# chongminggao/CIRS-codes

Hardware: AMD Instinct MI355X
Metric: simulator env-steps/s (collect + PPO update in the timed region), KuaishouEnv (higher is better)
Workload: dtype f32 (policy/tracker; rollout on the fp32 MFMA, PPO head products fp32-accurate from two fp16 pieces per operand (3 f16 MFMAs per product), fp32 accumulate) + f64 (env rewards, GAE)

## Files before the change

### cirs-codes_amd/csrc/internal.h

```cpp
#pragma once
#include "common.h"
#include "policy_kernels.h"

namespace cirs {

struct TrunkFuse {
    int on;
    cirs_policy_cfg cfg;
    cirs_policy_weights w;
    const uint8_t* skip;
    float* h2;
    float* value;
};

inline int device_cu_count() {
    static int cus = 0;
    if (cus == 0) {
        int dev = 0, n = 0;
        if (hipGetDevice(&dev) == hipSuccess && hipDeviceGetAttribute(&n, hipDeviceAttributeMultiprocessorCount, dev) == hipSuccess && n > 0) cus = n;
        else cus = 256;
    }
    return cus;
}

inline int head_tiles_per_chunk(int n_item_tiles, int n_row_blocks, int wgs_per_cu) {
    const long slots = (long)wgs_per_cu * device_cu_count();
    const int tpc = (int)(((long)n_item_tiles * n_row_blocks + slots - 1) / slots);
    return tpc < 4 ? 4 : tpc;
}

inline HeadGrid sampler_grid(int n_items, int n_pad) {
    HeadGrid g;
    const int tiles = (n_items + kTileN - 1) / kTileN;
    g.n_row_blocks = (n_pad / kTileM + 3) / 4;
    g.tiles_per_chunk = head_tiles_per_chunk(tiles, g.n_row_blocks, kSamplerWgsPerCu);
// ... 93 lines not shown
```

### cirs-codes_amd/csrc/policy.hip

```cpp
#include "policy_kernels.h"
#include "internal.h"

namespace cirs {

__global__ __launch_bounds__(256) void actor_merge_kernel(int n, int n_pad, int n_chunks, ActorPartialView pv,
                                                          const uint8_t* __restrict__ skip,
                                                          int64_t* __restrict__ act_out, float* __restrict__ logp_out) {
    const int lane = threadIdx.x & 63;
    const int j = blockIdx.x * 4 + (threadIdx.x >> 6);
    if (j >= n) return;
    if (skip && skip[j]) {
        if (lane == 0) {
            act_out[j] = -1;
            if (logp_out) logp_out[j] = 0.f;
        }
        return;
    }
    actor_merge_wave(j, lane, n_pad, n_chunks, pv, act_out, logp_out);
}

__global__ __launch_bounds__(256) void actor_shard_tuple_kernel(int n, int n_pad, int n_chunks, ActorPartialView pv,
                                                               const uint8_t* __restrict__ skip, float* __restrict__ out5) {
    const int lane = threadIdx.x & 63;
    const int j = blockIdx.x * 4 + (threadIdx.x >> 6);
// ... 92 lines not shown
    const long k = (long)blockIdx.x * blockDim.x + threadIdx.x;
    if (k >= n * q) return;
    const long r = k / q;
    const int c = (int)(k - r * q);
    const long id = idx[r];
    reinterpret_cast<float4*>(out)[k] = id < 0 ? make_float4(0.f, 0.f, 0.f, 0.f) : reinterpret_cast<const float4*>(table + (size_t)id * row_floats)[c];
}

static int validate_policy(const cirs_policy_cfg* cfg, const cirs_policy_weights* w) {
    CIRS_REQUIRE(cfg && w, "policy cfg/weights null");
    CIRS_REQUIRE(cfg->n_items > 0, "n_items must be positive");
    if (cfg->hidden != kH) return fail(CIRS_E_UNSUPPORTED, "this build supports hidden == 64 only");
    CIRS_REQUIRE(cfg->dim_state > 0 && cfg->dim_state <= 64, "dim_state must be in 1..64");
    CIRS_REQUIRE(w->w1 && w->b1 && w->w2 && w->b2 && w->wa && w->ba && w->wc && w->bc, "policy weight pointer null");
    return CIRS_OK;
}

}

extern "C" int64_t cirs_policy_workspace_bytes(const cirs_policy_cfg* cfg, int32_t n) {
    using namespace cirs;
    if (!cfg || n <= 0) return 0;
    return (int64_t)(ws_h2_floats(n) + 5 * ws_partial_elems(n, cfg->n_items) + ws_zstore_floats(n, cfg->n_items)) * 4 + 8192 + kTrkImgBytes +
           (int64_t)ws_rplanes_bytes(cfg->n_items) + 512;
}

extern "C" int cirs_actor_sample(const cirs_policy_cfg* cfg, const cirs_policy_weights* w, const float* state,
                                 int64_t state_stride, int32_t n, const float* gumbel, uint64_t seed,
                                 uint32_t rng_step, const int32_t* env_ids, const uint32_t* visited,
                                 const uint8_t* skip, int64_t* act_out, float* logp_out, float* value_out,
                                 void* workspace, int64_t workspace_bytes, void* stream) {
    using namespace cirs;
    if (int rc = validate_policy(cfg, w)) return rc;
    if (n <= 0) return CIRS_OK;
    CIRS_REQUIRE(state && act_out && workspace, "null state/act/workspace");
    CIRS_REQUIRE(state_stride >= cfg->dim_state, "state_stride < dim_state");
    if (n <= 0) return CIRS_OK;
    CIRS_REQUIRE(workspace_bytes >= cirs_policy_workspace_bytes(cfg, n), "workspace too small");
    hipStream_t s = (hipStream_t)stream;
    float* h2 = (float*)workspace;
    const int n_pad = n_pad_of(n);
    const HeadGrid hg = sampler_grid(cfg->n_items, n_pad);
    const int n_chunks = hg.n_chunks;
    ActorPartialView pv = partial_view(workspace, n, cfg->n_items);
    hipLaunchKernelGGL(trunk_kernel, dim3(cdiv(n, 4)), dim3(256), 0, s, *cfg, *w, state, (long)state_stride, n, skip, h2,
                       value_out, nullptr);
    CIRS_CHECK_LAUNCH("trunk_kernel");
    if (!gumbel) {
        const int nch = n_chunks_of(cfg->n_items);
        const int cpw = mass_chunks_per_wg(nch, hg.n_row_blocks);
        uint4* planes = ws_rplanes(workspace, workspace_bytes, cfg->n_items);
        if (int rc = build_rplanes(w->wa, cfg->n_items, planes, s)) return rc;
        hipLaunchKernelGGL(actor_mass_kernel, dim3(cdiv(nch, cpw), hg.n_row_blocks), dim3(kMassThreads), 0, s, *cfg, (const uint4*)planes, w->ba, (const float*)h2, n,
                           env_ids, visited, skip, pv.m, n_pad, cpw, 0, 0);
        CIRS_CHECK_LAUNCH("actor_mass_kernel");
        PickArgs pa{pv.m, n_pad, nch, w->wa, w->ba, h2, visited, cfg->n_items, 0, 0, seed, rng_step};
        hipLaunchKernelGGL(actor_pick_kernel, dim3(cdiv(n, 4)), dim3(256), 0, s, pa, n, env_ids, skip, act_out, logp_out, (float*)nullptr);
        CIRS_CHECK_LAUNCH("actor_pick_kernel");
        return CIRS_OK;
    }
    const dim3 grid(hg.grid_x, hg.n_row_blocks);
    hipLaunchKernelGGL(actor_head_kernel<kNoiseHarness>, grid, dim3(256), 0, s, *cfg, w->wa, w->ba, h2, n, gumbel, seed,
                       rng_step, env_ids, visited, skip, pv, n_pad, hg.tiles_per_chunk);
    CIRS_CHECK_LAUNCH("actor_head_kernel");
    hipLaunchKernelGGL(actor_merge_kernel, dim3(cdiv(n, 4)), dim3(256), 0, s, n, n_pad, n_chunks, pv, skip, act_out, logp_out);
    CIRS_CHECK_LAUNCH("actor_merge_kernel");
    return CIRS_OK;
}

namespace cirs {
static int greedy_head(const cirs_policy_cfg* cfg, const cirs_policy_weights* w, const float* state, int64_t state_stride, int32_t n,
                       const int32_t* env_ids, const uint32_t* visited, const uint8_t* skip, float* value_out, void* workspace, float* zfull,
                       hipStream_t s) {
    float* h2 = (float*)workspace;
    const int n_pad = n_pad_of(n);
    const HeadGrid hg = sampler_grid(cfg->n_items, n_pad);
// ... 75 lines not shown
                                         int64_t state_stride, int32_t n, uint64_t seed, uint32_t rng_step, const int32_t* env_ids,
                                         const uint32_t* visited, const uint8_t* skip, int32_t item_base, int32_t n_items_total,
                                         float* tuples_out, float* value_out, void* workspace, int64_t workspace_bytes, void* stream) {
    using namespace cirs;
    if (int rc = validate_policy(cfg_shard, w_shard)) return rc;
    if (n <= 0) return CIRS_OK;
    CIRS_REQUIRE(state && tuples_out && workspace, "null state/tuples/workspace");
    CIRS_REQUIRE(state_stride >= cfg_shard->dim_state, "state_stride < dim_state");
    CIRS_REQUIRE(item_base >= 0 && (item_base % CIRS_SAMPLER_CHUNK) == 0, "item_base must be a non-negative multiple of the sampler chunk (128 items)");
    CIRS_REQUIRE(n_items_total >= item_base + cfg_shard->n_items, "n_items_total < item_base + shard size");
    CIRS_REQUIRE(workspace_bytes >= cirs_policy_workspace_bytes(cfg_shard, n), "workspace too small");
    hipStream_t s = (hipStream_t)stream;
    float* h2 = (float*)workspace;
    const int n_pad = n_pad_of(n);
    const HeadGrid hg = sampler_grid(cfg_shard->n_items, n_pad);
    ActorPartialView pv = partial_view(workspace, n, cfg_shard->n_items);
    hipLaunchKernelGGL(trunk_kernel, dim3(cdiv(n, 4)), dim3(256), 0, s, *cfg_shard, *w_shard, state, (long)state_stride, n, skip, h2,
                       value_out, nullptr);
    CIRS_CHECK_LAUNCH("trunk_kernel");
    const int nch = n_chunks_of(cfg_shard->n_items);
    const int cpw = mass_chunks_per_wg(nch, hg.n_row_blocks);
    uint4* planes = ws_rplanes(workspace, workspace_bytes, cfg_shard->n_items);
    if (int rc = build_rplanes(w_shard->wa, cfg_shard->n_items, planes, s)) return rc;
    hipLaunchKernelGGL(actor_mass_kernel, dim3(cdiv(nch, cpw), hg.n_row_blocks), dim3(kMassThreads), 0, s, *cfg_shard, (const uint4*)planes, w_shard->ba,
                       (const float*)h2, n, env_ids, visited, skip, pv.m, n_pad, cpw, item_base, n_items_total);
    CIRS_CHECK_LAUNCH("actor_mass_kernel");
    PickArgs pa{pv.m, n_pad, nch, w_shard->wa, w_shard->ba, h2, visited, cfg_shard->n_items, item_base, n_items_total, seed, rng_step};
    hipLaunchKernelGGL(actor_pick_kernel, dim3(cdiv(n, 4)), dim3(256), 0, s, pa, n, env_ids, skip, (int64_t*)nullptr, (float*)nullptr, tuples_out);
    CIRS_CHECK_LAUNCH("actor_pick_kernel");
    return CIRS_OK;
}

extern "C" int cirs_actor_merge_shards(const float* tuples, int32_t n_shards, int32_t n, const uint8_t* skip, int64_t* act_out,
                                       float* logp_out, void* stream) {
    using namespace cirs;
    if (n <= 0) return CIRS_OK;
    CIRS_REQUIRE(tuples && act_out && n_shards > 0, "null tuples / act_out or n_shards <= 0");
    hipLaunchKernelGGL(actor_merge_shards_kernel, dim3(cdiv(n, 256)), dim3(256), 0, (hipStream_t)stream, tuples, n_shards, n, skip,
                       act_out, logp_out);
    CIRS_CHECK_LAUNCH("actor_merge_shards_kernel");
    return CIRS_OK;
}

extern "C" int cirs_gather_rows(const float* table, int32_t row_floats, const int64_t* idx, int64_t n, float* out, void* stream) {
    using namespace cirs;
    if (n <= 0) return CIRS_OK;
    CIRS_REQUIRE(table && idx && out, "null argument");
// ... 7 lines not shown
```

### cirs-codes_amd/csrc/policy_kernels.h

```cpp
#pragma once
#include "bf16x6.h"
#include "common.h"
#include "rng.h"

namespace cirs {

constexpr int kH = 64;
constexpr int kTileM = 32;
constexpr int kTileN = 32;
constexpr int kTilesPerChunk = 4;
constexpr int kChunkItems = kTileN * kTilesPerChunk;

typedef float f32x16 __attribute__((ext_vector_type(16)));

struct ActorPartialView {
    float* score;
    int32_t* idx;
    float* m;
    float* s;
    float* z;
};

__host__ __device__ inline int n_chunks_of(int n_items) { return (n_items + kChunkItems - 1) / kChunkItems; }
__host__ __device__ inline int n_pad_of(int n) { return ((n + kTileM - 1) / kTileM) * kTileM; }
// ... 283 lines not shown

constexpr int kMassRowB = 144;
constexpr int kMassPlaneB = kTileN * kMassRowB;
constexpr int kMassTileU4 = 512;
constexpr int kMassThreads = 512;
constexpr float kMassScWa = 256.f, kMassScH2 = 64.f, kMassScZ = kMassScWa * kMassScH2, kMassScZi = 1.0f / kMassScZ;
__host__ __device__ inline size_t ws_rplanes_bytes(int n_items) { return (size_t)n_chunks_of(n_items) * kTilesPerChunk * kMassTileU4 * 16; }

static __global__ __launch_bounds__(256) void wa_rplanes_kernel(const float* __restrict__ wa, int I, uint4* __restrict__ planes) {
    const int tid = threadIdx.x, tile = blockIdx.x;
    const int item = tile * kTileN + (tid >> 3), col = 8 * (tid & 7);
    typedef float rp_v4 __attribute__((ext_vector_type(4)));
    rp_v4 a = {0.f, 0.f, 0.f, 0.f}, b = a;
    if (item < I) {
        const rp_v4* src = reinterpret_cast<const rp_v4*>(wa + (size_t)item * kH + col);
        a = src[0]; b = src[1];
    }
    a *= kMassScWa; b *= kMassScWa;
    const Planes2 pl = split8h(a.x, a.y, a.z, a.w, b.x, b.y, b.z, b.w);
    uint4* out = planes + (size_t)tile * kMassTileU4;
    out[tid] = __builtin_bit_cast(uint4, pl.h); out[256 + tid] = __builtin_bit_cast(uint4, pl.l);
}

__device__ __forceinline__ void mass_split_hidden(const float* tile, int lo, int hi, Planes2 (&hz)[4]) {
    typedef float ms_v4 __attribute__((ext_vector_type(4)));
#pragma unroll
    for (int s4 = 0; s4 < 4; ++s4) {
        const ms_v4* src = reinterpret_cast<const ms_v4*>(&tile[lo * kLdsStride + 16 * s4 + 8 * hi]);
        const ms_v4 a = src[0] * kMassScH2, b = src[1] * kMassScH2;
        hz[s4] = split8h(a.x, a.y, a.z, a.w, b.x, b.y, b.z, b.w);
    }
}
__device__ __forceinline__ f32x16 mass_logits_tile(const unsigned char* tw, const float* sb, const Planes2 (&hz)[4], int lo, int hi) {
    Planes2 za[4];
#pragma unroll
    for (int s4 = 0; s4 < 4; ++s4) {
        const unsigned char* ap = tw + lo * kMassRowB + (16 * s4 + 8 * hi) * 2;
        za[s4].h = *reinterpret_cast<const f16x8*>(ap);
        za[s4].l = *reinterpret_cast<const f16x8*>(ap + kMassPlaneB);
    }
    f32x16 acc, accs, acct;
#pragma unroll
    for (int r = 0; r < 16; ++r) { acc[r] = sb[acc_row(r, hi)]; accs[r] = 0.f; acct[r] = 0.f; }
    mfma_f16x3_split2(za[0], hz[0], za[1], hz[1], acc, accs, acct);
    mfma_f16x3_split2(za[2], hz[2], za[3], hz[3], acc, accs, acct);
#pragma unroll
    for (int r = 0; r < 16; ++r) acc[r] = (acc[r] + (accs[r] + acct[r])) * kMassScZi;
    return acc;
}
__device__ __forceinline__ float mass_exp(float z, float nml) { return __builtin_amdgcn_exp2f(__builtin_fmaf(z, 1.4426950408889634f, nml)); }
__device__ __forceinline__ float mass_log(float s) { return __builtin_amdgcn_logf(s) * 0.6931471805599453f; }

#ifdef CIRS_MASS_PROF
static __device__ unsigned long long g_mass_prof[32];
#define CIRS_MSTAMP(K) do { if (blockIdx.x == 0 && blockIdx.y == 0 && threadIdx.x == 0) g_mass_prof[K] = __builtin_amdgcn_s_memtime(); } while (0)
#define CIRS_MSTAMP_IF(COND, K) do { if ((COND) && blockIdx.x == 0 && blockIdx.y == 0 && threadIdx.x == 0) g_mass_prof[K] = __builtin_amdgcn_s_memtime(); } while (0)
#else
#define CIRS_MSTAMP(K) do { } while (0)
#define CIRS_MSTAMP_IF(COND, K) do { } while (0)
#endif
static __global__ __launch_bounds__(512, 1) void actor_mass_kernel(cirs_policy_cfg cfg, const uint4* __restrict__ planes,
                                                                   const float* __restrict__ ba, const float* __restrict__ h2, int n,
                                                                   const int32_t* __restrict__ env_ids,
                                                                   const uint32_t* __restrict__ visited,
                                                                   const uint8_t* __restrict__ skip, float* __restrict__ lmass,
                                                                   int n_pad, int chunks_per_wg, int item_base = 0,
                                                                   int n_items_total = 0, int env_base = 0, float* __restrict__ zstore = nullptr) {
    __shared__ __attribute__((aligned(16))) unsigned char sW[2][kTilesPerChunk][2 * kMassPlaneB];
    __shared__ __attribute__((aligned(16))) float sB[2][kChunkItems];
    __shared__ float sM[4][2][kTileM];
    __shared__ float sS[4][2][kTileM];
    const int tid = threadIdx.x;
    CIRS_MSTAMP(0);
    const int lane = tid & 63, wv = tid >> 6;
    const int hi = lane >> 5, lo = lane & 31;
    const int rt = wv & 3, th = wv >> 2;
    const int row0 = (blockIdx.y * 4 + rt) * kTileM;
    const int I = cfg.n_items;
    const int I_tot = n_items_total > 0 ? n_items_total : I;
    const int vis_words = (I_tot + 31) / 32;
    const int n_chunks = n_chunks_of(I);
    const int c_begin = blockIdx.x * chunks_per_wg;
    const int c_end = min(n_chunks, c_begin + chunks_per_wg);
    const int dst_r = (tid >> 8) * kMassPlaneB + ((tid & 255) >> 3) * kMassRowB + (tid & 7) * 16;
    uint4 ga, gb4, gc, gd;
    float gb = 0.f;
    static_assert(kTilesPerChunk == 4, "the chunk staging names its four tiles");
#define CIRS_ISSUE(CHUNK)                                                                                  \
    do {                                                                                                   \
        const uint4* src_ = planes + (size_t)(CHUNK) * kTilesPerChunk * kMassTileU4 + tid;                 \
        ga = src_[0]; gb4 = src_[kMassTileU4]; gc = src_[2 * kMassTileU4]; gd = src_[3 * kMassTileU4];     \
        gb = ba[min((CHUNK) * kChunkItems + (tid & (kChunkItems - 1)), I - 1)];    \
    } while (0)
#define CIRS_COMMIT(BUF)                                                                                   \
    do {                                                                                                   \
        *reinterpret_cast<uint4*>(sW[BUF][0] + dst_r) = ga; *reinterpret_cast<uint4*>(sW[BUF][1] + dst_r) = gb4; \
        *reinterpret_cast<uint4*>(sW[BUF][2] + dst_r) = gc; *reinterpret_cast<uint4*>(sW[BUF][3] + dst_r) = gd;  \
        if (tid < kChunkItems) sB[BUF][tid] = gb_chunk * kChunkItems + tid < I ? kMassScZ * gb : 0.f;       \
    } while (0)
    int gb_chunk = min(c_begin, n_chunks - 1);
    CIRS_ISSUE(gb_chunk);
    const int jr = row0 + lo;
    const bool active = row0 < n_pad && jr < n && !(skip && skip[jr]);
    const bool wave_live = __ballot(active) != 0ull;
    const int e = active ? (env_ids ? env_ids[jr] : env_base + jr) : 0;
    Planes2 hz[4];
    {
        __shared__ __attribute__((aligned(16))) float sH[4][kTileM * kLdsStride];
        typedef float mass_v4 __attribute__((ext_vector_type(4)));
        if (th == 0 && wave_live) {
            mass_v4* st4 = reinterpret_cast<mass_v4*>(sH[rt]);
            mass_v4 t8[8];
#pragma unroll
            for (int q = 0; q < 8; ++q) {
                const int r = row0 + 4 * q + (lane >> 4);
                t8[q] = r < n ? *reinterpret_cast<const mass_v4*>(h2 + (size_t)r * kH + (lane & 15) * 4) : mass_v4{0.f, 0.f, 0.f, 0.f};
            }
#pragma unroll
            for (int q = 0; q < 8; ++q) st4[(4 * q + (lane >> 4)) * (kLdsStride / 4) + (lane & 15)] = t8[q];
        }
        __shared__ int s_any;
        if (tid == 0) s_any = 0;
        __syncthreads();
        if (wave_live && lane == 0) s_any = 1;
        __syncthreads();
        CIRS_MSTAMP(1);
        if (s_any == 0) {
            if (th == 0 && row0 < n_pad && hi == 0)
                for (int c = c_begin; c < c_end; ++c) lmass[(size_t)c * n_pad + jr] = -INFINITY;
            return;
// ... 85 lines not shown
#pragma unroll
            for (int q = 0; q < 32; ++q) sl += ex[q];
            float L = -INFINITY;
            const float so = __shfl_xor(sl, 32, CIRS_WAVE);
            if (M > -INFINITY) {
                const float S = hi == 0 ? sl + so : so + sl;
                L = M + mass_log(S);
            }
            if (row0 < n_pad && hi == 0) lmass[(size_t)c * n_pad + jr] = active ? L : -INFINITY;
        }
        CIRS_MSTAMP_IF(stamp_it, 13);
        asm volatile("" ::: "memory");
        if (more) {
            CIRS_COMMIT(buf ^ 1);
            __syncthreads();
        }
        CIRS_MSTAMP_IF(stamp_it, 14);
    }
    CIRS_MSTAMP(16);
#undef CIRS_ISSUE
#undef CIRS_COMMIT
}

static __global__ __launch_bounds__(1024) void actor_mass_small_kernel(cirs_policy_cfg cfg, const uint4* __restrict__ planes, const float* __restrict__ ba,
                                                                       const float* __restrict__ h2, int n, const uint32_t* __restrict__ visited,
                                                                       const uint8_t* __restrict__ skip, float* __restrict__ lmass, int n_pad, int env_base,
                                                                       float* __restrict__ zstore) {
    __shared__ __attribute__((aligned(16))) unsigned char sW[4][2 * kMassPlaneB];
    __shared__ __attribute__((aligned(16))) float sB[4][kTileN];
    __shared__ __attribute__((aligned(16))) float sH[4][kTileM * kLdsStride];
    __shared__ float sM[4][4][kTileM];
    __shared__ float sS[4][2][kTileM];
    static_assert(4 * 2 * kMassPlaneB + sizeof(float) * (4 * kTileN + 4 * kTileM * kLdsStride + 4 * 4 * kTileM + 4 * 2 * kTileM) <= 160 * 1024,
                  "actor_mass_small_kernel: LDS beyond gfx950's 160 KB");
    const int tid = threadIdx.x, n_thr = blockDim.x;
    const int lane = tid & 63, wv = tid >> 6;
    const int hi = lane >> 5, lo = lane & 31;
    const int rt = wv >> 2, tt = wv & 3;
    const int I = cfg.n_items, c = blockIdx.x;
    const int vis_words = (I + 31) / 32;
    typedef float mass_v4 __attribute__((ext_vector_type(4)));
    {
        const uint4* psrc = planes + (size_t)c * kTilesPerChunk * kMassTileU4;
        uint4 xr[8];
        mass_v4 hr[2];
#pragma unroll
        for (int q = 0; q < 8; ++q) xr[q] = psrc[min(tid + q * n_thr, 4 * kMassTileU4 - 1)];
#pragma unroll
        for (int q = 0; q < 2; ++q) {
            const int f = tid + q * n_thr, r = f >> 4, col4 = f & 15;
            hr[q] = (f < n_pad * (kH / 4) && r < n) ? *reinterpret_cast<const mass_v4*>(h2 + (size_t)r * kH + 4 * col4) : mass_v4{0.f, 0.f, 0.f, 0.f};
        }
        const float bq = tid < kChunkItems ? ba[min(c * kChunkItems + tid, I - 1)] : 0.f;
#pragma unroll
        for (int q = 0; q < 8; ++q) {
            const int f = tid + q * n_thr;
            if (f < 4 * kMassTileU4) {
                const int t = f / kMassTileU4, u = f - t * kMassTileU4, pl = u >> 8, v = u & 255;
                *reinterpret_cast<uint4*>(sW[t] + pl * kMassPlaneB + (v >> 3) * kMassRowB + (v & 7) * 16) = xr[q];
            }
        }
        if (tid < kChunkItems) sB[tid >> 5][tid & 31] = c * kChunkItems + tid < I ? kMassScZ * bq : 0.f;
#pragma unroll
        for (int q = 0; q < 2; ++q) {
            const int f = tid + q * n_thr, r = f >> 4, col4 = f & 15;
            if (f < n_pad * (kH / 4)) *reinterpret_cast<mass_v4*>(&sH[r >> 5][(r & 31) * kLdsStride + 4 * col4]) = hr[q];
        }
    }
    const int jr = rt * kTileM + lo;
    const bool active = jr < n && !(skip && skip[jr]);
    const int e = env_base + jr;
    const int tile0 = c * kChunkItems + tt * kTileN;
    const uint32_t vis = (visited && active && tile0 < I) ? visited[(size_t)e * vis_words + (tile0 >> 5)] : 0u;
    __syncthreads();
    f32x16 acc;
    {
        Planes2 hz[4];
        mass_split_hidden(sH[rt], lo, hi, hz);
        acc = mass_logits_tile(sW[tt], sB[tt], hz, lo, hi);
    }
    if (zstore && active) {
        float* zr = zstore + ((size_t)c * n_pad + jr) * kChunkItems + tt * kTileN + 4 * hi;
#pragma unroll
        for (int q = 0; q < 4; ++q) *reinterpret_cast<float4*>(zr + 8 * q) = make_float4(acc[4 * q], acc[4 * q + 1], acc[4 * q + 2], acc[4 * q + 3]);
    }
    float mloc = -INFINITY;
#pragma unroll
    for (int r = 0; r < 16; ++r) {
        const int il = (r & 3) + 8 * (r >> 2) + 4 * hi;
        const bool valid = tile0 + il < I && !((vis >> (il & 31)) & 1u);
        acc[r] = valid ? acc[r] : -INFINITY;
        mloc = fmaxf(mloc, acc[r]);
    }
    mloc = fmaxf(mloc, __shfl_xor(mloc, 32, CIRS_WAVE));
    if (hi == 0) sM[rt][tt][lo] = mloc;
    __syncthreads();
    const float M = fmaxf(fmaxf(sM[rt][0][lo], sM[rt][1][lo]), fmaxf(sM[rt][2][lo], sM[rt][3][lo]));
    float ex[16];
    if (M > -INFINITY) {
        const float nml = -M * 1.4426950408889634f;
#pragma unroll
        for (int r = 0; r < 16; ++r) ex[r] = mass_exp(acc[r], nml);
    } else {
// ... 354 lines not shown
```

### cirs-codes_amd/csrc/rollout.hip

```cpp
#include "env_kernels.h"
#include "internal.h"
#include "policy_kernels.h"

namespace cirs {

__global__ __launch_bounds__(256) void mark_visited_kernel(const int64_t* __restrict__ act, int n, int n_items,
                                                           uint32_t* __restrict__ visited) {
    const int j = blockIdx.x * blockDim.x + threadIdx.x;
    if (j >= n) return;
    const long a = act[j];
    if (a < 0) return;
    const int words = (n_items + 31) / 32;
    atomicOr(&visited[(size_t)j * words + (a >> 5)], 1u << (a & 31));
}

__global__ __launch_bounds__(256) void force_done_kernel(uint8_t* __restrict__ st_done, uint8_t* __restrict__ done_row,
                                                         const int64_t* __restrict__ act, int n, int force_done) {
    const int j = blockIdx.x * blockDim.x + threadIdx.x;
    if (j >= n) return;
    if (act[j] < 0) return;
    st_done[j] = (uint8_t)force_done;
    done_row[j] = (uint8_t)force_done;
}

__global__ __launch_bounds__(256) void online_pairs_kernel(const int32_t* __restrict__ env_user, const int64_t* __restrict__ act, int n,
                                                           cirs_online_reward o) {
    const int j = blockIdx.x * blockDim.x + threadIdx.x;
    if (j >= n) return;
    const long a = act[j] < 0 ? 0 : act[j];
    o.uid_buf[j] = o.raw_uid[env_user[j]];
    o.pid_buf[j] = o.raw_pid[a];
#pragma unroll
    for (int q = 0; q < 4; ++q) o.feat_buf[(size_t)j * 4 + q] = o.item_feats[(size_t)a * 4 + q];
    o.dur_buf[j] = o.item_dur[a];
}

static inline int64_t sampler_ws_bytes(const cirs_policy_cfg* cfg, int n) {
    return (int64_t)(ws_h2_floats(n) + 5 * ws_partial_elems(n, cfg->n_items)) * 4;
}

}

static int rollout_impl(const cirs_env_cfg* env_cfg, const cirs_env_tables* env_tab, cirs_env_state* env_st,
                        const cirs_tracker_cfg* trk_cfg, const cirs_tracker_weights* trk_w, cirs_tracker_state* trk_st,
                        const cirs_policy_cfg* pol_cfg, const cirs_policy_weights* pol_w, const cirs_traj* traj, int32_t n_env,
                        int32_t t_begin, int32_t t_end, uint64_t seed, uint32_t rng_base, uint32_t* visited, int32_t force_length,
                        const cirs_online_reward* online, const float* gumbel, void* workspace, int64_t workspace_bytes, void* stream,
                        const cirs_redraw* redraw = nullptr, const int32_t* init_users = nullptr, bool greedy = false);

extern "C" int cirs_rollout_collect(const cirs_env_cfg* env_cfg, const cirs_env_tables* env_tab, cirs_env_state* env_st,
                                    const cirs_tracker_cfg* trk_cfg, const cirs_tracker_weights* trk_w, cirs_tracker_state* trk_st,
                                    const cirs_policy_cfg* pol_cfg, const cirs_policy_weights* pol_w, const cirs_traj* traj, int32_t n_env,
                                    const int32_t* users, uint64_t seed, uint32_t rng_base, uint32_t* visited, int32_t force_length, void* workspace,
                                    int64_t workspace_bytes, void* stream) {
    CIRS_REQUIRE(env_cfg && env_st && users && workspace && n_env > 0, "cirs_rollout_collect: null argument");
    CIRS_REQUIRE(workspace_bytes >= (int64_t)sizeof(int64_t) * n_env, "workspace too small");
    CIRS_REQUIRE(env_st->user && env_st->turn && env_st->done && env_st->hist_action && env_st->cum_reward, "env state has null field");
    return rollout_impl(env_cfg, env_tab, env_st, trk_cfg, trk_w, trk_st, pol_cfg, pol_w, traj, n_env, 0, env_cfg->max_turn, seed, rng_base, visited, force_length,
                        nullptr, nullptr, workspace, workspace_bytes, stream, nullptr, users);
}

// ... 200 lines not shown
    CIRS_REQUIRE(pol_cfg->hidden == kH && pol_cfg->dim_state == S && pol_cfg->n_items == env_cfg->n_items, "policy/env/tracker shape mismatch");
    CIRS_REQUIRE(pol_w->w1 && pol_w->b1 && pol_w->w2 && pol_w->b2 && pol_w->wa && pol_w->ba && pol_w->wc && pol_w->bc, "policy weight pointer null");
    CIRS_REQUIRE(workspace_bytes >= cirs_policy_workspace_bytes(pol_cfg, n_env), "workspace too small");
    CIRS_REQUIRE(env_tab->item_cats && (env_tab->normed_mat || !env_cfg->simulated) && (env_tab->mat || env_cfg->simulated), "env tables incomplete");
    if (t_begin >= t_end) return CIRS_OK;
    float* img = (float*)((char*)workspace + ((workspace_bytes - kTrkImgBytes) & ~(int64_t)255));
    uint4* rplanes = ws_rplanes(workspace, workspace_bytes, pol_cfg->n_items);
    if (int rc = pack_tracker_image(trk_cfg, trk_w, pol_w, S, img, s, pol_w->wa, pol_cfg->n_items, merge_tail ? nullptr : rplanes, init_users ? env_cfg : nullptr, env_st,
                                    init_users, n_env, (int64_t*)workspace))
        return rc;
    const int n_pad = n_pad_of(n_env);
    const int n_mass_chunks = n_chunks_of(pol_cfg->n_items);
    float* h2 = (float*)workspace;
    const ActorPartialView pv = partial_view(workspace, n_env, pol_cfg->n_items);
    const HeadGrid hg = sampler_grid(pol_cfg->n_items, n_pad);
    const int cpw = mass_chunks_per_wg(n_mass_chunks, hg.n_row_blocks);
    float* zstore = nullptr;
    if (!merge_tail && ws_zstore_floats(n_env, pol_cfg->n_items) > 0) {
        const char* ev = getenv("CIRS_ROLLOUT_ZSTORE");
        if (ev ? atoi(ev) != 0 : true) zstore = (float*)((char*)workspace + ((sampler_ws_bytes(pol_cfg, n_env) + 255) & ~(int64_t)255));
    }
    const char* ms_ev = getenv("CIRS_ROLLOUT_MASS_SMALL");
    const bool mass_small = (ms_ev ? atoi(ms_ev) != 0 : true) && !merge_tail && n_pad <= 128;
    const uint8_t* done_all = (const uint8_t*)env_st->done;
    auto redraw_state = [&](int t, bool with_trunk) -> int {
        cirs_tracker_cfg cfg_t = *trk_cfg;
        cfg_t.dropout_seed = redraw->dropout_seed;
        cfg_t.drop_env_base = (int32_t)(redraw->env_base0 + (int64_t)t * redraw->env_stride);
        const size_t start = (size_t)B * t * (t + 1) / 2;
        TrunkFuse tf{};
        if (with_trunk) { tf.on = 1; tf.cfg = *pol_cfg; tf.w = *pol_w; tf.skip = done_all; tf.h2 = h2; tf.value = traj->value + (size_t)t * B; }
        int fused = 0;
        if (int rc = tracker_prefix_states_trunk(&cfg_t, trk_w, trk_st, redraw->row_env + start, redraw->row_t + start, redraw->offsets + (size_t)t * B,
                                                 redraw->lens + (size_t)t * B, (int32_t)(B * (t + 1)), traj->obs + (size_t)t * B * S, S, redraw->workspace,
                                                 redraw->workspace_bytes, stream, &tf, &fused))
            return rc;
        if (with_trunk && !fused) {
            hipLaunchKernelGGL(trunk_kernel, dim3(cdiv(n_env, 4)), dim3(256), 0, s, *pol_cfg, *pol_w, traj->obs + (size_t)t * B * S, (long)S, n_env, done_all, h2,
                               traj->value + (size_t)t * B, (float*)nullptr);
            CIRS_CHECK_LAUNCH("trunk_kernel");
        }
        return CIRS_OK;
    };
    bool first_trunk_done = false;
    if (init_users) {
        TrunkFuse tf0{};
        if (!redraw) {
            tf0.on = 1; tf0.cfg = *pol_cfg; tf0.w = *pol_w; tf0.skip = nullptr; tf0.h2 = h2; tf0.value = traj->value + (size_t)t_begin * B;
            first_trunk_done = true;
        }
        if (int rc = tracker_step_internal(trk_cfg, trk_w, trk_st, init_users, nullptr, nullptr, nullptr, nullptr, n_env, traj->obs + (size_t)t_begin * B * S, S, &tf0, s,
                                           nullptr, img))
            return rc;
    }
    if (redraw) { if (int rc = redraw_state(t_begin, true)) return rc; }
    if (!redraw && !first_trunk_done)
        hipLaunchKernelGGL(trunk_kernel, dim3(cdiv(n_env, 4)), dim3(256), 0, s, *pol_cfg, *pol_w, traj->obs + (size_t)t_begin * B * S, (long)S, n_env, done_all,
                           h2, traj->value + (size_t)t_begin * B, (float*)nullptr);
    CIRS_CHECK_LAUNCH("trunk_kernel");
    for (int t = t_begin; t < t_end; ++t) {
        const float* gum_t = gumbel ? gumbel + (size_t)t * B * pol_cfg->n_items : (const float*)nullptr;
        float* obs_n = traj->obs + (size_t)(t + 1) * B * S;
        int64_t* act_t = traj->act + (size_t)t * B;
        double* rew_t = traj->rew + (size_t)t * B;
        uint8_t* done_t = traj->done + (size_t)t * B;
        if (gum_t) {
            CIRS_PROF_LAUNCH(3, s, hipLaunchKernelGGL(actor_head_kernel<kNoiseHarness>, dim3(hg.grid_x, hg.n_row_blocks), dim3(256), 0, s, *pol_cfg,
                                                      pol_w->wa, pol_w->ba, (const float*)h2, n_env, gum_t, seed,
                                                      rng_base + (uint32_t)t, (const int32_t*)nullptr, (const uint32_t*)visited,
                                                      done_all, pv, n_pad, hg.tiles_per_chunk));
        } else if (greedy) {
            CIRS_PROF_LAUNCH(3, s, hipLaunchKernelGGL(actor_head_kernel<kNoiseNone>, dim3(hg.grid_x, hg.n_row_blocks), dim3(256), 0, s, *pol_cfg,
                                                      pol_w->wa, pol_w->ba, (const float*)h2, n_env, (const float*)nullptr, (uint64_t)0, 0u,
                                                      (const int32_t*)nullptr, (const uint32_t*)visited, done_all, pv, n_pad, hg.tiles_per_chunk));
        } else if (mass_small) {
            CIRS_PROF_LAUNCH(3, s, hipLaunchKernelGGL(actor_mass_small_kernel, dim3(n_mass_chunks), dim3(n_pad / kTileM * 256), 0, s, *pol_cfg, (const uint4*)rplanes,
                                                      pol_w->ba, (const float*)h2, n_env, (const uint32_t*)visited, done_all, pv.m, n_pad, 0, zstore));
        } else {
            CIRS_PROF_LAUNCH(3, s, hipLaunchKernelGGL(actor_mass_kernel, dim3(cdiv(n_mass_chunks, cpw), hg.n_row_blocks), dim3(kMassThreads), 0,
                                                      s, *pol_cfg, (const uint4*)rplanes, pol_w->ba, (const float*)h2, n_env, (const int32_t*)nullptr,
                                                      (const uint32_t*)visited, done_all, pv.m, n_pad, cpw, 0, 0, 0, zstore));
        }
        CIRS_CHECK_LAUNCH("sampler kernel");
        TrunkFuse tf{};
        if (t + 1 < t_end && !redraw) {
            tf.on = 1; tf.cfg = *pol_cfg; tf.w = *pol_w; tf.skip = done_all; tf.h2 = h2;
            tf.value = traj->value + (size_t)(t + 1) * B;
        }
        TailFuse tl{};
        tl.on = 1; tl.cfg = *env_cfg; tl.tab = *env_tab; tl.st = *env_st; tl.n_pad = n_pad; tl.n_chunks = hg.n_chunks; tl.pv = pv;
        tl.env_base = 0;
        tl.visited = visited; tl.force_length = force_length;
        if (!merge_tail) {
            tl.pick_on = 1;
            tl.pick = PickArgs{pv.m, n_pad, n_mass_chunks, pol_w->wa, pol_w->ba, h2, visited, pol_cfg->n_items, 0, 0, seed, rng_base + (uint32_t)t, zstore};
        }
        tl.force_done = (t + 1 >= force_length) ? 1 : 0;
        tl.slot_only = redraw && (t + 1 < t_end || t + 1 < trk_cfg->max_len) ? 1 : 0;
        tl.act_out = act_t; tl.logp_out = traj->logp + (size_t)t * B; tl.rew_out = rew_t; tl.done_out = done_t;
        tl.ctr_out = traj->ctr + (size_t)t * B;
        if (int rc = tracker_step_internal(trk_cfg, trk_w, trk_st, nullptr, act_t, rew_t, nullptr, nullptr, n_env, obs_n, S, &tf, s, &tl, img))
            return rc;
        if (redraw && (t + 1 < t_end || t + 1 < trk_cfg->max_len)) {
            if (int rc = redraw_state(t + 1, t + 1 < t_end)) return rc;
        }
    }
    return CIRS_OK;
}

#ifdef CIRS_MASS_PROF
// ... 5 lines not shown
```

### cirs-codes_amd/csrc/tracker.hip

```cpp
#include <hip/hip_runtime.h>
#ifdef CIRS_TRK_PROF
namespace cirs { extern __device__ unsigned long long g_trk_prof[64]; }
#define CIRS_PICK_STAMP(K) do { if (blockIdx.x == 0 && threadIdx.x == 0) cirs::g_trk_prof[K] = __builtin_amdgcn_s_memtime(); } while (0)
#endif
#include "internal.h"
#include "policy_kernels.h"
#include "env_kernels.h"

namespace cirs {

constexpr int kD = 32;
constexpr int kHid = 128;

template <int K>
__device__ __forceinline__ float dot_row(const float* __restrict__ wrow, const float* xs, float acc) {
    const float4* w4 = reinterpret_cast<const float4*>(wrow);
#pragma unroll
    for (int k4 = 0; k4 < K / 4; ++k4) {
        const float4 w = w4[k4];
        acc = __builtin_fmaf(w.x, xs[4 * k4 + 0], acc);
        acc = __builtin_fmaf(w.y, xs[4 * k4 + 1], acc);
        acc = __builtin_fmaf(w.z, xs[4 * k4 + 2], acc);
        acc = __builtin_fmaf(w.w, xs[4 * k4 + 3], acc);
    }
// ... 57 lines not shown
                                                           cirs_tracker_state st, const int32_t* __restrict__ users,
                                                           const int64_t* __restrict__ items,
                                                           const double* __restrict__ rew,
                                                           const int32_t* __restrict__ env_ids,
                                                           const uint8_t* __restrict__ skip, int n,
                                                           float* __restrict__ state_out, long state_stride,
                                                           int lpad, TrunkFuse tf, TailFuse tl, const float* __restrict__ img,
                                                           TrkImg IL) {
    extern __shared__ __attribute__((aligned(16))) float smem[];
    constexpr int HD = kD / NHEAD;
    const int lane = threadIdx.x & 63, wv = threadIdx.x >> 6;
    const int nwv = blockDim.x >> 6;
    const int j = blockIdx.x * nwv + wv;
    CIRS_STAMP(0);
    kernarg_warm<sizeof(cirs_tracker_cfg) + sizeof(cirs_tracker_weights) + sizeof(cirs_tracker_state) + sizeof(TrunkFuse) + sizeof(TailFuse) +
                 sizeof(TrkImg) + 64>();
    CIRS_STAMP(1);
    if (j >= n) return;
#define CIRS_TRUNK_ZERO()                                                  \
    do {                                                                   \
        if (tf.on) {                                                       \
            tf.h2[(size_t)j * kH + lane] = 0.f;                            \
            if (lane == 0 && tf.value) tf.value[j] = 0.f;                  \
        }                                                                  \
    } while (0)
    const bool is_init = users != nullptr;
    const int o32 = lane & (kD - 1);
    const int e = env_ids ? env_ids[j] : (tl.on ? tl.env_base + j : j);
    RowRegs<kD> gp;
    float g_r = 0.f, gbias = 0.f;
#define CIRS_GATE_PREFETCH()                                                                   \
    do {                                                                                       \
        if (!is_init) {                                                                        \
            if (IMG) {                                                                         \
                g_r = img[IL.gate_r + o32]; gbias = img[IL.gate_b + o32];                      \
                gp = wrow<kD, true>(img, IL.gate_p, kD, nullptr, 0, o32, 0);                   \
            } else {                                                                           \
                const float* gw = w.gate_w + (size_t)o32 * (kD + 1);    \
                g_r = gw[0]; gbias = w.gate_b[o32];                                            \
                _Pragma("unroll") for (int k4 = 0; k4 < kD / 4; ++k4)                          \
                    gp.q[k4] = make_float4(gw[1 + 4 * k4], gw[2 + 4 * k4], gw[3 + 4 * k4], gw[4 + 4 * k4]); \
            }                                                                                  \
        }                                                                                      \
    } while (0)
    const int B = cfg.n_env, L = cfg.max_len;
    float* base = smem + (size_t)wv * (6 * kD + kHid + NHEAD * lpad);
// ... 362 lines not shown
            const int S = tf.cfg.dim_state;
            __builtin_amdgcn_wave_barrier();
            float acc = tb1;
#pragma unroll
            for (int k = 0; k < kD; ++k)
                if (k < S) acc = __builtin_fmaf(tw1[k], txs[k], acc);
            ths[lane] = fmaxf(acc, 0.f);
            __builtin_amdgcn_wave_barrier();
            const float h2v = fmaxf(dot_pre<kH>(tw2, ths, tb2), 0.f);
            tf.h2[(size_t)j * kH + lane] = h2v;
            __builtin_amdgcn_wave_barrier();
            txs[lane] = h2v;
            ths[lane] = twc;
            __builtin_amdgcn_wave_barrier();
            if (lane == 0 && tf.value) {
                float v = tbc;
#pragma unroll
                for (int k = 0; k < kH; ++k) v = __builtin_fmaf(ths[k], txs[k], v);
                tf.value[j] = v;
            }
        } else {
            trunk_compute(tf.cfg, tf.w, txs, ths, lane, j, tf.h2, tf.value, nullptr);
        }
    }
    CIRS_STAMP(19);
#undef CIRS_TRUNK_ZERO
#undef CIRS_KV_PREFETCH
#undef CIRS_DROP
}

struct SetupExtra {
    int n_img, n_rp, n_reset;
    const float* wa; int n_items; uint4* planes;
    cirs_env_cfg ecfg; cirs_env_state est; const int32_t* users; int n_env; int64_t* obs_scratch;
};
__global__ __launch_bounds__(256) void pack_tracker_image_kernel(cirs_tracker_cfg cfg, cirs_tracker_weights w, cirs_policy_weights pol, int S,
                                                                 TrkImg L, float* __restrict__ img, SetupExtra x) {
    if ((int)blockIdx.x >= x.n_img) {
        const int b = (int)blockIdx.x - x.n_img;
        if (b < x.n_rp) {
            const int tid = threadIdx.x, item = b * kTileN + (tid >> 3), col = 8 * (tid & 7);
            typedef float rp_v4 __attribute__((ext_vector_type(4)));
            rp_v4 a = {0.f, 0.f, 0.f, 0.f}, bb = a;
            if (item < x.n_items) {
                const rp_v4* src = reinterpret_cast<const rp_v4*>(x.wa + (size_t)item * kH + col);
                a = src[0]; bb = src[1];
// ... 171 lines not shown
```

Baseline: 5.936 million.

## Precompute fp16 hidden-state planes in tracker trunk for mass kernels

The tracker's fused trunk now also writes the scaled, split fp16 high/low planes of each row's h2 into a new workspace buffer laid out per 32-row tile. The mass and small-mass sampler kernels are templated so they can load these planes directly into registers instead of staging h2 through LDS and splitting it per block. The full-mass variant can also exit early when no wave in the workgroup has a live row. This adds workspace, extra stores in the tracker and a new layout coupling between kernels, with an env var to fall back to the fp32 path.

```diff
diff --git a/cirs-codes_amd/csrc/internal.h b/cirs-codes_amd/csrc/internal.h
--- a/cirs-codes_amd/csrc/internal.h
+++ b/cirs-codes_amd/csrc/internal.h
@@ -11,6 +11,7 @@
     const uint8_t* skip;
     float* h2;
     float* value;
+    uint4* hz;
 };
 
 inline int device_cu_count() {
diff --git a/cirs-codes_amd/csrc/policy.hip b/cirs-codes_amd/csrc/policy.hip
--- a/cirs-codes_amd/csrc/policy.hip
+++ b/cirs-codes_amd/csrc/policy.hip
@@ -138,7 +138,7 @@
     using namespace cirs;
     if (!cfg || n <= 0) return 0;
     return (int64_t)(ws_h2_floats(n) + 5 * ws_partial_elems(n, cfg->n_items) + ws_zstore_floats(n, cfg->n_items)) * 4 + 8192 + kTrkImgBytes +
-           (int64_t)ws_rplanes_bytes(cfg->n_items) + 512;
+           (int64_t)ws_rplanes_bytes(cfg->n_items) + 512 + (int64_t)ws_h2planes_bytes(n) + 256;
 }
 
 extern "C" int cirs_actor_sample(const cirs_policy_cfg* cfg, const cirs_policy_weights* w, const float* state,
@@ -167,7 +167,7 @@
         const int cpw = mass_chunks_per_wg(nch, hg.n_row_blocks);
         uint4* planes = ws_rplanes(workspace, workspace_bytes, cfg->n_items);
         if (int rc = build_rplanes(w->wa, cfg->n_items, planes, s)) return rc;
-        hipLaunchKernelGGL(actor_mass_kernel, dim3(cdiv(nch, cpw), hg.n_row_blocks), dim3(kMassThreads), 0, s, *cfg, (const uint4*)planes, w->ba, (const float*)h2, n,
+        hipLaunchKernelGGL(actor_mass_kernel<false>, dim3(cdiv(nch, cpw), hg.n_row_blocks), dim3(kMassThreads), 0, s, *cfg, (const uint4*)planes, w->ba, (const float*)h2, n,
                            env_ids, visited, skip, pv.m, n_pad, cpw, 0, 0);
         CIRS_CHECK_LAUNCH("actor_mass_kernel");
         PickArgs pa{pv.m, n_pad, nch, w->wa, w->ba, h2, visited, cfg->n_items, 0, 0, seed, rng_step};
@@ -289,7 +289,7 @@
     const int cpw = mass_chunks_per_wg(nch, hg.n_row_blocks);
     uint4* planes = ws_rplanes(workspace, workspace_bytes, cfg_shard->n_items);
     if (int rc = build_rplanes(w_shard->wa, cfg_shard->n_items, planes, s)) return rc;
-    hipLaunchKernelGGL(actor_mass_kernel, dim3(cdiv(nch, cpw), hg.n_row_blocks), dim3(kMassThreads), 0, s, *cfg_shard, (const uint4*)planes, w_shard->ba,
+    hipLaunchKernelGGL(actor_mass_kernel<false>, dim3(cdiv(nch, cpw), hg.n_row_blocks), dim3(kMassThreads), 0, s, *cfg_shard, (const uint4*)planes, w_shard->ba,
                        (const float*)h2, n, env_ids, visited, skip, pv.m, n_pad, cpw, item_base, n_items_total);
     CIRS_CHECK_LAUNCH("actor_mass_kernel");
     PickArgs pa{pv.m, n_pad, nch, w_shard->wa, w_shard->ba, h2, visited, cfg_shard->n_items, item_base, n_items_total, seed, rng_step};
diff --git a/cirs-codes_amd/csrc/policy_kernels.h b/cirs-codes_amd/csrc/policy_kernels.h
--- a/cirs-codes_amd/csrc/policy_kernels.h
+++ b/cirs-codes_amd/csrc/policy_kernels.h
@@ -329,13 +329,35 @@
     out[tid] = __builtin_bit_cast(uint4, pl.h); out[256 + tid] = __builtin_bit_cast(uint4, pl.l);
 }
 
+__device__ __forceinline__ Planes2 mass_split8(const float* p8) {
+    typedef float ms_v4 __attribute__((ext_vector_type(4)));
+    const ms_v4* src = reinterpret_cast<const ms_v4*>(p8);
+    const ms_v4 a = src[0] * kMassScH2, b = src[1] * kMassScH2;
+    return split8h(a.x, a.y, a.z, a.w, b.x, b.y, b.z, b.w);
+}
 __device__ __forceinline__ void mass_split_hidden(const float* tile, int lo, int hi, Planes2 (&hz)[4]) {
-    typedef float ms_v4 __attribute__((ext_vector_type(4)));
+#pragma unroll
+    for (int s4 = 0; s4 < 4; ++s4) hz[s4] = mass_split8(&tile[lo * kLdsStride + 16 * s4 + 8 * hi]);
+}
+constexpr int kHzTileU4 = 512;
+__host__ inline size_t ws_h2planes_bytes(int n) { return (size_t)n_pad_of(n) * 256; }
+__host__ inline size_t ws_h2planes_offset(int n, int n_items) { return ((ws_h2_floats(n) + 5 * ws_partial_elems(n, n_items)) * 4 + 255) & ~(size_t)255; }
+__device__ __forceinline__ void mass_row_planes_store(const float* row64, int j, int lane, uint4* __restrict__ hzp) {
+    if (lane < 8) {
+        const Planes2 pl = mass_split8(row64 + 8 * lane);
+        uint4* dst = hzp + (size_t)(j >> 5) * kHzTileU4 + (lane >> 1) * 128 + (lane & 1) * 32 + (j & 31);
+        dst[0] = __builtin_bit_cast(uint4, pl.h); dst[64] = __builtin_bit_cast(uint4, pl.l);
+    }
+}
+__device__ __forceinline__ void mass_row_planes_zero(int j, int lane, uint4* __restrict__ hzp) {
+    if (lane < 16) hzp[(size_t)(j >> 5) * kHzTileU4 + (lane >> 1) * 64 + (lane & 1) * 32 + (j & 31)] = make_uint4(0u, 0u, 0u, 0u);
+}
+__device__ __forceinline__ void mass_load_planes(const uint4* __restrict__ hzp, int tile, int lane, Planes2 (&hz)[4]) {
+    const uint4* src = hzp + (size_t)tile * kHzTileU4 + lane;
 #pragma unroll
     for (int s4 = 0; s4 < 4; ++s4) {
-        const ms_v4* src = reinterpret_cast<const ms_v4*>(&tile[lo * kLdsStride + 16 * s4 + 8 * hi]);
-        const ms_v4 a = src[0] * kMassScH2, b = src[1] * kMassScH2;
-        hz[s4] = split8h(a.x, a.y, a.z, a.w, b.x, b.y, b.z, b.w);
+        hz[s4].h = __builtin_bit_cast(f16x8, src[s4 * 128]);
+        hz[s4].l = __builtin_bit_cast(f16x8, src[s4 * 128 + 64]);
     }
 }
 __device__ __forceinline__ f32x16 mass_logits_tile(const unsigned char* tw, const float* sb, const Planes2 (&hz)[4], int lo, int hi) {
@@ -366,6 +388,7 @@
 #define CIRS_MSTAMP(K) do { } while (0)
 #define CIRS_MSTAMP_IF(COND, K) do { } while (0)
 #endif
+template <bool HP>
 static __global__ __launch_bounds__(512, 1) void actor_mass_kernel(cirs_policy_cfg cfg, const uint4* __restrict__ planes,
                                                                    const float* __restrict__ ba, const float* __restrict__ h2, int n,
                                                                    const int32_t* __restrict__ env_ids,
@@ -405,14 +428,30 @@
         *reinterpret_cast<uint4*>(sW[BUF][2] + dst_r) = gc; *reinterpret_cast<uint4*>(sW[BUF][3] + dst_r) = gd;  \
         if (tid < kChunkItems) sB[BUF][tid] = gb_chunk * kChunkItems + tid < I ? kMassScZ * gb : 0.f;       \
     } while (0)
+    const int jr = row0 + lo;
+    Planes2 hz[4];
+    bool row_done = false;
+    if constexpr (HP) {
+        row_done = skip[min(jr, n - 1)] != 0;
+        mass_load_planes(reinterpret_cast<const uint4*>(h2), min(row0, n_pad - kTileM) / kTileM, lane, hz);
+    }
     int gb_chunk = min(c_begin, n_chunks - 1);
     CIRS_ISSUE(gb_chunk);
-    const int jr = row0 + lo;
-    const bool active = row0 < n_pad && jr < n && !(skip && skip[jr]);
+    const bool active = row0 < n_pad && jr < n && !(HP ? row_done : (skip && skip[jr]));
     const bool wave_live = __ballot(active) != 0ull;
     const int e = active ? (env_ids ? env_ids[jr] : env_base + jr) : 0;
-    Planes2 hz[4];
-    {
+    if constexpr (HP) {
+        __shared__ __attribute__((aligned(16))) int s_live[kMassThreads / 64];
+        if (lane == 0) s_live[wv] = wave_live ? 1 : 0;
+        __syncthreads();
+        CIRS_MSTAMP(1);
+        const int4 v0 = *reinterpret_cast<const int4*>(&s_live[0]), v1 = *reinterpret_cast<const int4*>(&s_live[4]);
+        if (((v0.x | v0.y) | (v0.z | v0.w) | (v1.x | v1.y) | (v1.z | v1.w)) == 0) {
+            if (th == 0 && row0 < n_pad && hi == 0)
+                for (int c = c_begin; c < c_end; ++c) lmass[(size_t)c * n_pad + jr] = -INFINITY;
+            return;
+        }
+    } else {
         __shared__ __attribute__((aligned(16))) float sH[4][kTileM * kLdsStride];
         typedef float mass_v4 __attribute__((ext_vector_type(4)));
         if (th == 0 && wave_live) {
@@ -544,6 +583,7 @@
 #undef CIRS_COMMIT
 }
 
+template <bool HP>
 static __global__ __launch_bounds__(1024) void actor_mass_small_kernel(cirs_policy_cfg cfg, const uint4* __restrict__ planes, const float* __restrict__ ba,
                                                                        const float* __restrict__ h2, int n, const uint32_t* __restrict__ visited,
                                                                        const uint8_t* __restrict__ skip, float* __restrict__ lmass, int n_pad, int env_base,
@@ -562,16 +602,21 @@
     const int I = cfg.n_items, c = blockIdx.x;
     const int vis_words = (I + 31) / 32;
     typedef float mass_v4 __attribute__((ext_vector_type(4)));
+    Planes2 hz[4];
     {
         const uint4* psrc = planes + (size_t)c * kTilesPerChunk * kMassTileU4;
         uint4 xr[8];
         mass_v4 hr[2];
 #pragma unroll
         for (int q = 0; q < 8; ++q) xr[q] = psrc[min(tid + q * n_thr, 4 * kMassTileU4 - 1)];
-#pragma unroll
-        for (int q = 0; q < 2; ++q) {
-            const int f = tid + q * n_thr, r = f >> 4, col4 = f & 15;
-            hr[q] = (f < n_pad * (kH / 4) && r < n) ? *reinterpret_cast<const mass_v4*>(h2 + (size_t)r * kH + 4 * col4) : mass_v4{0.f, 0.f, 0.f, 0.f};
+        if constexpr (HP) {
+            mass_load_planes(reinterpret_cast<const uint4*>(h2), rt, lane, hz);
+        } else {
+#pragma unroll
+            for (int q = 0; q < 2; ++q) {
+                const int f = tid + q * n_thr, r = f >> 4, col4 = f & 15;
+                hr[q] = (f < n_pad * (kH / 4) && r < n) ? *reinterpret_cast<const mass_v4*>(h2 + (size_t)r * kH + 4 * col4) : mass_v4{0.f, 0.f, 0.f, 0.f};
+            }
         }
         const float bq = tid < kChunkItems ? ba[min(c * kChunkItems + tid, I - 1)] : 0.f;
 #pragma unroll
@@ -583,10 +628,12 @@
             }
         }
         if (tid < kChunkItems) sB[tid >> 5][tid & 31] = c * kChunkItems + tid < I ? kMassScZ * bq : 0.f;
-#pragma unroll
-        for (int q = 0; q < 2; ++q) {
-            const int f = tid + q * n_thr, r = f >> 4, col4 = f & 15;
-            if (f < n_pad * (kH / 4)) *reinterpret_cast<mass_v4*>(&sH[r >> 5][(r & 31) * kLdsStride + 4 * col4]) = hr[q];
+        if constexpr (!HP) {
+#pragma unroll
+            for (int q = 0; q < 2; ++q) {
+                const int f = tid + q * n_thr, r = f >> 4, col4 = f & 15;
+                if (f < n_pad * (kH / 4)) *reinterpret_cast<mass_v4*>(&sH[r >> 5][(r & 31) * kLdsStride + 4 * col4]) = hr[q];
+            }
         }
     }
     const int jr = rt * kTileM + lo;
@@ -595,12 +642,8 @@
     const int tile0 = c * kChunkItems + tt * kTileN;
     const uint32_t vis = (visited && active && tile0 < I) ? visited[(size_t)e * vis_words + (tile0 >> 5)] : 0u;
     __syncthreads();
-    f32x16 acc;
-    {
-        Planes2 hz[4];
-        mass_split_hidden(sH[rt], lo, hi, hz);
-        acc = mass_logits_tile(sW[tt], sB[tt], hz, lo, hi);
-    }
+    if constexpr (!HP) mass_split_hidden(sH[rt], lo, hi, hz);
+    f32x16 acc = mass_logits_tile(sW[tt], sB[tt], hz, lo, hi);
     if (zstore && active) {
         float* zr = zstore + ((size_t)c * n_pad + jr) * kChunkItems + tt * kTileN + 4 * hi;
 #pragma unroll
diff --git a/cirs-codes_amd/csrc/rollout.hip b/cirs-codes_amd/csrc/rollout.hip
--- a/cirs-codes_amd/csrc/rollout.hip
+++ b/cirs-codes_amd/csrc/rollout.hip
@@ -36,7 +36,7 @@
 }
 
 static inline int64_t sampler_ws_bytes(const cirs_policy_cfg* cfg, int n) {
-    return (int64_t)(ws_h2_floats(n) + 5 * ws_partial_elems(n, cfg->n_items)) * 4;
+    return (int64_t)(ws_h2planes_offset(n, cfg->n_items) + ws_h2planes_bytes(n));
 }
 
 }
@@ -283,6 +283,8 @@
     }
     const char* ms_ev = getenv("CIRS_ROLLOUT_MASS_SMALL");
     const bool mass_small = (ms_ev ? atoi(ms_ev) != 0 : true) && !merge_tail && n_pad <= 128;
+    const char* hf_ev = getenv("CIRS_ROLLOUT_H2_FP32");
+    uint4* hzp = (!merge_tail && !redraw && !(hf_ev && atoi(hf_ev) != 0)) ? (uint4*)((char*)workspace + ws_h2planes_offset(n_env, pol_cfg->n_items)) : nullptr;
     const uint8_t* done_all = (const uint8_t*)env_st->done;
     auto redraw_state = [&](int t, bool with_trunk) -> int {
         cirs_tracker_cfg cfg_t = *trk_cfg;
@@ -308,6 +310,7 @@
         TrunkFuse tf0{};
         if (!redraw) {
             tf0.on = 1; tf0.cfg = *pol_cfg; tf0.w = *pol_w; tf0.skip = nullptr; tf0.h2 = h2; tf0.value = traj->value + (size_t)t_begin * B;
+            tf0.hz = hzp;
             first_trunk_done = true;
         }
         if (int rc = tracker_step_internal(trk_cfg, trk_w, trk_st, init_users, nullptr, nullptr, nullptr, nullptr, n_env, traj->obs + (size_t)t_begin * B * S, S, &tf0, s,
@@ -334,19 +337,29 @@
             CIRS_PROF_LAUNCH(3, s, hipLaunchKernelGGL(actor_head_kernel<kNoiseNone>, dim3(hg.grid_x, hg.n_row_blocks), dim3(256), 0, s, *pol_cfg,
                                                       pol_w->wa, pol_w->ba, (const float*)h2, n_env, (const float*)nullptr, (uint64_t)0, 0u,
                                                       (const int32_t*)nullptr, (const uint32_t*)visited, done_all, pv, n_pad, hg.tiles_per_chunk));
-        } else if (mass_small) {
-            CIRS_PROF_LAUNCH(3, s, hipLaunchKernelGGL(actor_mass_small_kernel, dim3(n_mass_chunks), dim3(n_pad / kTileM * 256), 0, s, *pol_cfg, (const uint4*)rplanes,
-                                                      pol_w->ba, (const float*)h2, n_env, (const uint32_t*)visited, done_all, pv.m, n_pad, 0, zstore));
         } else {
-            CIRS_PROF_LAUNCH(3, s, hipLaunchKernelGGL(actor_mass_kernel, dim3(cdiv(n_mass_chunks, cpw), hg.n_row_blocks), dim3(kMassThreads), 0,
-                                                      s, *pol_cfg, (const uint4*)rplanes, pol_w->ba, (const float*)h2, n_env, (const int32_t*)nullptr,
-                                                      (const uint32_t*)visited, done_all, pv.m, n_pad, cpw, 0, 0, 0, zstore));
+            const bool hp = hzp && (t > t_begin || first_trunk_done);
+            const float* hsrc = hp ? (const float*)hzp : (const float*)h2;
+#define CIRS_MASS_LAUNCH(HP)                                                                                                                                       \
+            do {                                                                                                                                                   \
+                if (mass_small)                                                         \
+                    CIRS_PROF_LAUNCH(3, s, hipLaunchKernelGGL(actor_mass_small_kernel<HP>, dim3(n_mass_chunks), dim3(n_pad / kTileM * 256), 0, s, *pol_cfg,         \
+                                                              (const uint4*)rplanes, pol_w->ba, hsrc, n_env, (const uint32_t*)visited, done_all, pv.m, n_pad, 0,    \
+                                                              zstore));                                                                                            \
+                else                                                                                                                                               \
+                    CIRS_PROF_LAUNCH(3, s, hipLaunchKernelGGL(actor_mass_kernel<HP>, dim3(cdiv(n_mass_chunks, cpw), hg.n_row_blocks), dim3(kMassThreads), 0, s,     \
+                                                              *pol_cfg, (const uint4*)rplanes, pol_w->ba, hsrc, n_env, (const int32_t*)nullptr,                     \
+                                                              (const uint32_t*)visited, done_all, pv.m, n_pad, cpw, 0, 0, 0, zstore));                              \
+            } while (0)
+            if (hp) CIRS_MASS_LAUNCH(true); else CIRS_MASS_LAUNCH(false);
+#undef CIRS_MASS_LAUNCH
         }
         CIRS_CHECK_LAUNCH("sampler kernel");
         TrunkFuse tf{};
         if (t + 1 < t_end && !redraw) {
             tf.on = 1; tf.cfg = *pol_cfg; tf.w = *pol_w; tf.skip = done_all; tf.h2 = h2;
             tf.value = traj->value + (size_t)(t + 1) * B;
+            tf.hz = hzp;
         }
         TailFuse tl{};
         tl.on = 1; tl.cfg = *env_cfg; tl.tab = *env_tab; tl.st = *env_st; tl.n_pad = n_pad; tl.n_chunks = hg.n_chunks; tl.pv = pv;
diff --git a/cirs-codes_amd/csrc/tracker.hip b/cirs-codes_amd/csrc/tracker.hip
--- a/cirs-codes_amd/csrc/tracker.hip
+++ b/cirs-codes_amd/csrc/tracker.hip
@@ -103,6 +103,7 @@
         if (tf.on) {                                                       \
             tf.h2[(size_t)j * kH + lane] = 0.f;                            \
             if (lane == 0 && tf.value) tf.value[j] = 0.f;                  \
+            if (tf.hz) mass_row_planes_zero(j, lane, tf.hz);               \
         }                                                                  \
     } while (0)
     const bool is_init = users != nullptr;
@@ -511,6 +512,7 @@
         } else {
             trunk_compute(tf.cfg, tf.w, txs, ths, lane, j, tf.h2, tf.value, nullptr);
         }
+        if (tf.hz) mass_row_planes_store(txs, j, lane, tf.hz);
     }
     CIRS_STAMP(19);
 #undef CIRS_TRUNK_ZERO
```

Measured after the change: 5.993 million, median of 6. No clear change (+1.0%).
